# ru1ven/KeypointFusion

Hardware: AMD Instinct MI355X
Metric: RGB-D img/sec fwd (B=64, 256x256) (higher is better)
Workload: dtype f32; 1 GPU; KPFusion-convnext-tiny, depth+RGB UNet backbones forward, B=64/GPU 256x256 f32 (BASELINE configs[1]); batch_per_gpu=64, global_batch=64, input=256x256, parallelism=dp1 (batch shards, no collective)

## Files before the change

include/kpf.h:

```cpp
#ifndef KPF_H
#define KPF_H

#ifdef __cplusplus
extern "C" {
#endif

#define KPF_OK 0
#define KPF_EINVAL (-1)
#define KPF_ELAUNCH (-2)

#define KPF_DT_F32 0
#define KPF_DT_BF16 1
#define KPF_DT_F16 2
#define KPF_DT_F32_MMA_BF16 8
#define KPF_DT_F32_MMA_F16 9

#define KPF_ACT_RELU 1u
#define KPF_ACT_GELU 2u
#define KPF_RES_ADD 4u
#define KPF_RES_GAMMA 8u
#define KPF_RELU_AFTER_RES 16u
#define KPF_ACT_LEAKY 64u
#define KPF_IN_SPLIT 128u
#define KPF_W_SPLIT 512u
#define KPF_OUT_SPLIT 256u
#define KPF_OUT_NCHW 32u
#define KPF_ACT_GELU_SAVE 2048u
#define KPF_MMA_BF16 8192u
#define KPF_MMA_F16 16384u
#define KPF_PRO_LN 4096u
#define KPF_RES_GELU_GRAD 1024u

typedef struct kpf_conv_desc {
  int B, IH, IW, Cin;
  int in_ld, in_coff;
  int OH, OW, N;
  int KH, KW, sh, sw, ph, pw;
  int Kp;
  int out_ld, out_coff;
  int res_ld, res_coff;
  unsigned flags;
  float w_unscale;
  int tile_cfg;
  int groups;
  long w_gstride;
} kpf_conv_desc;

int kpf_conv2d_f32(const kpf_conv_desc* d, const float* in, const float* w, const float* bias,
                   const float* pro_scale, const float* pro_shift, const float* gamma, const float* res,
                   float* out, void* stream);

int kpf_dwconv7_ln_f32(const float* x, const float* w_dw, const float* b_dw, const float* ln_w, const float* ln_b,
                       float* y, int B, int H, int W, int C, float eps, void* stream);

int kpf_convnext_mlp_f32(const float* y, const float* x, const float* w1, const float* b1, const float* w2, const float* b2,
                         const float* gamma, float* out, long M, int C, void* stream);
int kpf_convnext_mlp_supported(int C);
int kpf_convnext_mlp_split_f32(const float* y_split, const float* x, const float* w1_split, const float* b1, float w1_unscale,
                               const float* w2_split_perm, const float* b2, float w2_unscale, const float* gamma, float* out, long M,
                               int C, void* stream);
int kpf_convnext_mlp_split_supported(int C);
int kpf_convnext_mlp_h16(const void* y, const void* x, const void* w1, const float* b1, const void* w2_chunks, const float* b2,
                         const float* gamma, void* out, long M, int C, int dtype, void* stream);
int kpf_convnext_mlp_h16_supported(int C);

int kpf_dwconv7_stats_h16(const void* x, const float* w_dw, const float* b_dw, void* y, float* stats, int B, int H, int W, int C, int dtype,
                          void* stream);
int kpf_dwconv7_stats_supported(int H, int W, int C);
long kpf_dwconv7_stats_floats(int B, int H, int W, int C);
int kpf_ln_apply_stats_h16(void* y, const float* stats, const float* ln_w, const float* ln_b, long rows, int C, float eps, int dtype, void* stream);
int kpf_ln_stats_merge(const float* stats, float* mean_rstd, long rows, int C, float eps, void* stream);

int kpf_layernorm_f32(const float* x, const float* w, const float* b, float* y, long rows, int C, float eps, void* stream);

int kpf_dwconv7_ln_split_f32(const float* x, const float* w_dw, const float* b_dw, const float* ln_w, const float* ln_b, float* y,
                             int B, int H, int W, int C, float eps, void* stream);
int kpf_layernorm_split_f32(const float* x, const float* w, const float* b, float* y, long rows, int C, float eps, void* stream);

int kpf_upsample2x_f32(const float* src, float* dst, int B, int H, int W, int C, int dst_ld, int dst_coff, void* stream);

int kpf_nchw_to_nhwc_f32(const float* src, float* dst, int B, int C, int H, int W, int Cpad, void* stream);

int kpf_nhwc_to_nchw_f32(const float* src, float* dst, int B, int C, int H, int W, int src_ld, int src_coff, void* stream);

int kpf_maxpool3x3s2_f32(const float* src, float* dst, int B, int H, int W, int C, void* stream);


int kpf_inv3x3_f32(const float* M, float* Minv, int B, int fused, void* stream);

int kpf_offset2joint_f32(const float* offset, const float* depth, const float* center, const float* Minv, const float* cube,
                         const float* cam, float* joint_uvd, float* joint_xyz, int B, int S, int F, float kernel,
                         int img_size, int flip, void* stream);

int kpf_img2pcl_top4_f32(const float* pcl, const float* depth, const float* center, const float* Minv, const float* cube,
                         const float* cam, float* closeness, int* index, float* img_xyz, int B, int N, int S, int F,
                         int img_size, int flip, void* stream);

int kpf_point_assemble_f32(const float* feat_d, const float* feat_rgb, const float* offset, const float* pcl,
                           const float* joint_xyz, const float* closeness, const int* index, float* A1, float* A2, int B,
                           int N, int P, float kernel, void* stream);

int kpf_softmax_pool_f32(const float* A1, const float* X, const float* joint_xyz, float* JA, int B, int N, void* stream);

// ... 368 lines not shown
                      int* bounds, double* M64, void* stream);

int kpf_prep_pcl_sample(const float* img, const float* center, const double* M64, const double* cube, const double* cam, const long long* seed, int B, int S,
                        int n, float* pcl, int* pcl_index, int* pcl_count, float* cand_pts, void* stream);

int kpf_prep_uncrop_f32(const float* joints, const float* center, const float* M, const float* cube, const float* cam, int B, int J, float* crop_px,
                        float* frame_px, void* stream);

int kpf_prep_set_stamps(void* stamps64 );

int kpf_eval_errors_f32(const float* const* stages, int S, const float* gt, const float* cube, const int* score_index, int B, int J, int Jsel, float* err,
                        void* stream);

int kpf_eval_accumulate(const float* err, const unsigned char* valid, const double* thresholds, int S, int B, int Jsel, int T, long long* n_samples,
                        long long* n_batches, double* sum_err, double* sum_pa, double* sum_batch_mean, double* sum_batch_pa_mean, long long* pck,
                        long long* pck_pa, void* stream);

int kpf_prep_crop_u16_indexed(const unsigned char* rgb, const unsigned short* depth, const int* frame_index, int F, const double* bbox, const double* cam,
                              const double* cube, int B, int Hs, int Ws, int x0, int y0, int H, int W, int S, float* img, float* img_rgb, float* center, float* M,
                              float* cube_out, float* cam_para, double* com, int* bounds, double* M64, void* stream);

int kpf_track_step_f32(const float* joints, const float* center, const float* M, const float* cube, const float* cam_para, const int* pcl_count, int B, int J,
                       int frame_w, int frame_h, float expansion, long long seed_stride, double* bbox, long long* seed, int* lost, float* crop_px,
                       float* frame_px, float* cam_mm, double* bbox_used, int* status, void* stream);

int kpf_prep_annot_u16(const unsigned char* rgb, const unsigned short* depth, const int* frame_index, int F, const float* joints_mm, const float* cam32,
                       const float* center_xyz, const unsigned char* mirror, const double* cube, int B, int J, int Hs, int Ws, int x0, int y0, int H, int W, int S,
                       float* img, float* img_rgb, float* center, float* M, float* cube_out, float* cam_para, double* com, int* bounds, double* M64, float* joint,
                       float* joint_img, double* cam64, void* stream);

int kpf_prep_uncrop_mirror_f32(const float* joints, const float* center, const float* M, const float* cube, const float* cam, const unsigned char* mirror,
                               int frame_w, int B, int J, float* crop_px, float* frame_px, void* stream);

int kpf_prep_augment_u16(const unsigned char* rgb, const unsigned short* depth, const int* frame_index, int F, const float* joints_mm, const float* cam32,
                         const float* center_xyz, const unsigned char* mirror, const double* cube, const int* mode, const double* off, const double* sc,
                         const double* rot, const double* rot_cs, const double* color, int B, int J, int Hs, int Ws, int x0, int y0, int H, int W, int S,
                         float* img, float* img_rgb, float* center, float* M, float* cube_out, float* cam_para, double* com, int* bounds, double* M64,
                         float* joint, float* joint_img, double* cam64, double* cube64, int* aug_status, void* stream);

int kpf_prep_aug_draw(long long* seed, int B, double sigma_com, double sigma_sc, double rot_range, double color_factor, long long seed_stride, int* mode,
                      double* off, double* sc, double* rot, double* rot_cs, double* color, void* stream);

int kpf_eval_mesh_f32(const float* pred, const float* gt, const float* pred_origin, const float* gt_origin, const double* thresholds, int T,
                      const double* f_thresholds, int Tf, int B, int V, float* err, float* nn, int* nn_idx, double* mean_err, int* pck_cnt, int* f_cnt,
                      void* stream);

int kpf_eval_mesh_accumulate(const float* err, const double* mean_err, const int* pck_cnt, const int* f_cnt, const unsigned char* valid, int B, int V, int T,
                             int Tf, long long* n_samples, long long* n_batches, double* sum_mean_err, double* sum_vert, long long* pck, double* sum_f,
                             void* stream);

int kpf_conv_num_tile_cfgs(void);

const char* kpf_last_error(void);
#define KPF_ABI_VERSION 32
int kpf_abi_version(void);

#ifdef __cplusplus
}
#endif
#endif
```

keypointfusion_amd/csrc/kpf_common.h:

```cpp
#pragma once
#include <hip/hip_runtime.h>
#include <stdarg.h>
#include <stdio.h>

#include "../../include/kpf.h"

typedef float f32x4 __attribute__((ext_vector_type(4)));
typedef _Float16 f16x4 __attribute__((ext_vector_type(4)));
typedef _Float16 f16x8 __attribute__((ext_vector_type(8)));

void kpf_set_error(const char* fmt, ...);

#define KPF_REQUIRE(cond, ...)    \
  do {                            \
    if (!(cond)) {                \
      kpf_set_error(__VA_ARGS__); \
      return KPF_EINVAL;          \
    }                             \
  } while (0)

static inline int kpf_check_launch(const char* what) {
  hipError_t e = hipGetLastError();
  if (e != hipSuccess) {
    kpf_set_error("%s: %s", what, hipGetErrorString(e));
    return KPF_ELAUNCH;
  }
  return KPF_OK;
}

#include <atomic>
constexpr int KPF_MAX_DEVICES = 64;
static inline bool kpf_raise_lds_limit(const void* kern, std::atomic<bool>* done) {
  int dev = 0;
  if (hipGetDevice(&dev) != hipSuccess || dev < 0 || dev >= KPF_MAX_DEVICES) return false;
  if (done[dev].load(std::memory_order_acquire)) return true;
  if (hipFuncSetAttribute(kern, hipFuncAttributeMaxDynamicSharedMemorySize, 160 * 1024) != hipSuccess) return false;
  done[dev].store(true, std::memory_order_release);
  return true;
}

void kpf_dw7_select_wgrad(int B, int H, int W, int C, bool raise_refused, kpf_dw7_plan* p, unsigned* grid_x);

static inline bool kpf_aligned16(const void* p) { return (reinterpret_cast<uintptr_t>(p) & 15u) == 0; }

__device__ __forceinline__ float wave_sum(float v) {
#pragma unroll
  for (int o = 32; o > 0; o >>= 1) v += __shfl_xor(v, o, 64);
  return v;
}
__device__ __forceinline__ float wave_max(float v) {
#pragma unroll
  for (int o = 32; o > 0; o >>= 1) v = fmaxf(v, __shfl_xor(v, o, 64));
  return v;
}

__host__ __device__ __forceinline__ unsigned hash32(unsigned x) {
  x ^= x >> 16;
  x *= 0x7feb352dU;
  x ^= x >> 15;
  x *= 0x846ca68bU;
  x ^= x >> 16;
  return x;
}

__device__ __forceinline__ void kpf_uncrop_joint(const float* __restrict__ j, const float* __restrict__ center, const float* __restrict__ M,
                                                 const float* __restrict__ cube, const float* __restrict__ cam, float* crop3, float* frame3,
                                                 double mirror_w = -1.0) {
#pragma clang fp contract(off)
  double m[9];
  for (int k = 0; k < 9; ++k) m[k] = (double)M[k];
  const double x = (double)j[0] * ((double)cube[0] / 2.0) + (double)center[0];
  const double y = (double)j[1] * ((double)cube[1] / 2.0) + (double)center[1];
  const double z = (double)j[2] * ((double)cube[2] / 2.0) + (double)center[2];
  const double u = x * (double)cam[0] / z + (double)cam[2], v = y * (double)cam[1] / z + (double)cam[3];
  const double cu = u * m[0] + v * m[1] + m[2], cv = u * m[3] + v * m[4] + m[5];
  crop3[0] = (float)cu;
  crop3[1] = (float)cv;
  crop3[2] = (float)z;
  const double c00 = m[4] * m[8] - m[5] * m[7], c01 = m[2] * m[7] - m[1] * m[8], c02 = m[1] * m[5] - m[2] * m[4];
  const double c10 = m[5] * m[6] - m[3] * m[8], c11 = m[0] * m[8] - m[2] * m[6], c12 = m[2] * m[3] - m[0] * m[5];
  const double c20 = m[3] * m[7] - m[4] * m[6], c21 = m[1] * m[6] - m[0] * m[7], c22 = m[0] * m[4] - m[1] * m[3];
  const double det = m[0] * c00 + m[1] * c10 + m[2] * c20;
  const double h0 = (cu * c00 + cv * c01 + c02) / det, h1 = (cu * c10 + cv * c11 + c12) / det, h2 = (cu * c20 + cv * c21 + c22) / det;
  const double fu = h0 / h2;
  frame3[0] = (float)(mirror_w >= 0.0 ? (mirror_w - 1.0) - fu : fu);
  frame3[1] = (float)(h1 / h2);
  frame3[2] = (float)z;
}

typedef __bf16 bf16_t;
typedef _Float16 f16_t;
typedef __bf16 bf16x4 __attribute__((ext_vector_type(4)));
typedef __bf16 bf16x8 __attribute__((ext_vector_type(8)));

// ... 39 lines not shown
```

keypointfusion_amd/csrc/kpf_conv.hip:

```cpp
#include "kpf_common.h"
#include <stdlib.h>
#include <type_traits>

namespace {

struct ConvArgs {
  const float* in;
  const float* w;
  const float* bias;
  const float* ps;
  const float* pt;
  const float* gamma;
  const float* res;
  float* out;
  int M, N, K, Kp;
  int IH, IW, Cin, in_ld, in_coff;
  int OH, OW, ohow, KH, KW, sh, sw, ph, pw;
  int out_ld, out_coff, res_ld, res_coff;
  const float* zero;
  float w_unscale;
  unsigned flags;
  int tilesN, nblk;
  int vec;
  int dbg;
// ... 1418 lines not shown
  KPF_REQUIRE(!(fl & KPF_RES_GELU_GRAD) || ((fl & KPF_RES_ADD) && !(fl & (KPF_RES_GAMMA | KPF_RELU_AFTER_RES | KPF_OUT_NCHW))), "kpf_conv2d_f32: RES_GELU_GRAD goes with RES_ADD alone");
  KPF_REQUIRE(!(fl & KPF_ACT_GELU_SAVE) || ((fl & KPF_ACT_GELU) && !(fl & (KPF_RES_ADD | KPF_OUT_NCHW)) && res && kpf_aligned16(res) && d->res_coff >= 0 && d->res_coff + d->N <= d->res_ld),
              "kpf_conv2d_f32: ACT_GELU_SAVE goes with ACT_GELU and a second output buffer in the res slot (res_ld / res_coff describe it)");
  KPF_REQUIRE((long)d->B * d->OH * d->OW < (1l << 31) && (long)d->B * d->IH * d->IW < (1l << 31), "kpf_conv2d_f32: too many pixels");

  ConvArgs a;
  a.in = in; a.w = w; a.bias = bias; a.ps = pro_scale; a.pt = pro_shift; a.gamma = gamma; a.res = res; a.out = out;
  a.M = d->B * d->OH * d->OW; a.N = d->N; a.K = d->KH * d->KW * d->Cin; a.Kp = d->Kp;
  a.IH = d->IH; a.IW = d->IW; a.Cin = d->Cin; a.in_ld = d->in_ld; a.in_coff = d->in_coff;
  a.OH = d->OH; a.OW = d->OW; a.ohow = d->OH * d->OW; a.KH = d->KH; a.KW = d->KW;
  a.sh = d->sh; a.sw = d->sw; a.ph = d->ph; a.pw = d->pw;
  a.out_ld = d->out_ld; a.out_coff = d->out_coff; a.res_ld = d->res_ld; a.res_coff = d->res_coff;
  {
    static const float* zero_of_dev[64] = {nullptr};
    int dev = 0;
    if (hipGetDevice(&dev) != hipSuccess || dev < 0 || dev >= 64) dev = 0;
    if (!zero_of_dev[dev]) {
      void* p = nullptr;
      if (hipGetSymbolAddress(&p, HIP_SYMBOL(kpf_zero16)) != hipSuccess || !p) {
        kpf_set_error("kpf_conv2d_f32: cannot resolve the zero page");
        return KPF_ELAUNCH;
      }
      zero_of_dev[dev] = static_cast<const float*>(p);
    }
    a.zero = zero_of_dev[dev];
  }
  a.flags = fl; a.tilesN = 0; a.nblk = 0; a.dbg = 0; a.skew = 0; a.st_policy = 0;
  {
    static const int st_mb = []() { const char* e = getenv("KPF_F32_ST_MB"); return e ? atoi(e) : 0; }();
    if (st_mb > 0 && (long)d->B * d->OH * d->OW * d->N * 4 >= (long)st_mb * 1000000) a.st_policy = 2;
  }
  a.w_unscale = (fl & (KPF_IN_SPLIT | KPF_W_SPLIT)) ? d->w_unscale : 1.0f;
  if (fl & (KPF_IN_SPLIT | KPF_W_SPLIT))
    KPF_REQUIRE(d->w_unscale > 0.f && d->Cin % 32 == 0 && d->in_coff % 4 == 0, "kpf_conv2d_f32: split operands need w_unscale > 0 and Cin %% 32 == 0 (Cin=%d)", d->Cin);
  if (fl & KPF_IN_SPLIT) KPF_REQUIRE(d->in_coff % 32 == 0 && d->in_ld % 32 == 0 && !pro_scale, "kpf_conv2d_f32: split activations need in_ld, in_coff multiples of 32 and no operand prologue");
  if (fl & KPF_OUT_SPLIT)
    KPF_REQUIRE(d->N % 32 == 0 && d->out_coff % 32 == 0 && d->out_ld % 32 == 0 && !(fl & KPF_OUT_NCHW),
                "kpf_conv2d_f32: split output needs N, out_ld, out_coff multiples of 32 (N=%d ld=%d coff=%d)", d->N, d->out_ld, d->out_coff);
  a.vec = (d->out_ld % 4 == 0 && d->out_coff % 4 == 0 && (!(fl & KPF_RES_ADD) || (d->res_ld % 4 == 0 && d->res_coff % 4 == 0))) ? 1 : 0;
  a.groups = d->groups > 1 ? d->groups : 1; a.g_in = a.g_out = 0; a.g_w = 0;
  if (a.groups > 1) {
    KPF_REQUIRE(!(fl & (KPF_RES_GAMMA | KPF_OUT_NCHW | KPF_IN_SPLIT | KPF_W_SPLIT | KPF_OUT_SPLIT)) && !pro_scale && d->w_gstride % 4 == 0,
                "kpf_conv2d_f32: a grouped launch takes no layer scale / prologue / NCHW output / split operands, and needs w_gstride %% 4 == 0");
    KPF_REQUIRE(d->in_coff + d->groups * d->Cin <= d->in_ld && d->out_coff + d->groups * d->N <= d->out_ld, "kpf_conv2d_f32: the groups' channel slices exceed the pixel stride");
    KPF_REQUIRE(!(fl & (KPF_RES_ADD | KPF_ACT_GELU_SAVE)) || d->res_coff + d->groups * d->N <= d->res_ld,
                "kpf_conv2d_f32: the groups' residual / saved pre-activation slices exceed the pixel stride");
    a.g_in = d->Cin; a.g_out = d->N; a.g_w = d->w_gstride;
    if ((d->out_coff + d->N) % 4 || ((fl & KPF_RES_ADD) && (d->res_coff + d->N) % 4)) a.vec = 0;
  }
  const bool is1x1 = d->KH == 1 && d->KW == 1 && d->sh == 1 && d->sw == 1 && d->ph == 0 && d->pw == 0 &&
                     d->IH == d->OH && d->IW == d->OW && d->Cin % 32 == 0 && d->Kp == d->Cin;
  hipStream_t st = reinterpret_cast<hipStream_t>(stream);

  int best = 0;
  double bc = 1e30;
  static const int forced = []() { const char* e = getenv("KPF_FORCE_CFG"); return e ? atoi(e) : -1; }();
  for (int i = 0; i < (int)(sizeof(kCfgs) / sizeof(kCfgs[0])); ++i) {
    const double c = cfg_cost(kCfgs[i], a.M, a.N, a.groups);
    if (c < bc) { bc = c; best = i; }
  }
  const bool f32_arith = !(fl & (KPF_IN_SPLIT | KPF_W_SPLIT));
  const bool gelu1x1 = f32_arith && is1x1 && (fl & KPF_ACT_GELU) && !(fl & KPF_ACT_GELU_SAVE) && !pro_scale && d->groups <= 1;
  if (gelu1x1 && a.M >= 1024 && a.N >= 512) {
    auto rounds_cost = [&](int bm, int bn, double pen) { return (double)((((long)(a.M + bm - 1) / bm) * ((a.N + bn - 1) / bn) + 255) / 256) * bm * bn * pen; };
    const double c0 = rounds_cost(128, 128, 1.00), c8 = rounds_cost(256, 128, 0.97);
    best = c0 <= c8 ? 0 : 8;
  }
  if (f32_arith && best < 9 && a.Kp >= 512) {
    const long bb = ((a.M + kCfgs[best].bm - 1) / kCfgs[best].bm) * ((a.N + kCfgs[best].bn - 1) / kCfgs[best].bn) * a.groups;
    if (bb < 256 && (long)((a.M + 31) / 32) * ((a.N + 63) / 64) * a.groups >= 512) best = 7;
  }
  if ((fl & (KPF_IN_SPLIT | KPF_W_SPLIT)) && !(fl & KPF_RES_ADD) && !pro_scale && (best == 0 || best == 8)) best = 13;
  if ((fl & (KPF_IN_SPLIT | KPF_W_SPLIT)) && !pro_scale && a.Kp >= 1024) {
    const long blocks = ((a.M + kCfgs[best < 9 ? best : 0].bm - 1) / kCfgs[best < 9 ? best : 0].bm) *
                        ((a.N + kCfgs[best < 9 ? best : 0].bn - 1) / kCfgs[best < 9 ? best : 0].bn);
    const long blocks64 = ((a.M + 63) / 64) * ((a.N + 63) / 64);
    if (best < 9 && blocks <= 512 && blocks64 >= 512) best = 16;
  }
  if (forced >= 0) best = forced;
  if (d->tile_cfg > 0) {
    KPF_REQUIRE(d->tile_cfg <= KPF_NUM_TILE_CFGS, "kpf_conv2d_f32: tile_cfg %d out of range", d->tile_cfg);
    best = d->tile_cfg - 1;
  }
#ifdef KPF_FAST_BUILD
  return launch_cfg<4, 4, 2, 2>(a, is1x1, st);
#else
  switch (best) {
    case 0: return launch_cfg<4, 4, 2, 2>(a, is1x1, st);
    case 1: return launch_cfg<4, 3, 2, 2>(a, is1x1, st);
    case 2: return launch_cfg<2, 4, 4, 1>(a, is1x1, st);
    case 3: return launch_cfg<4, 3, 4, 1>(a, is1x1, st);
    case 4: return launch_cfg<2, 7, 4, 1>(a, is1x1, st);
    case 5: return launch_cfg<2, 4, 2, 2>(a, is1x1, st);
    case 6: return launch_cfg<2, 2, 2, 2>(a, is1x1, st);
    case 8: return launch_cfg<4, 4, 4, 2>(a, is1x1, st);
    case 9: return launch_cfg<4, 4, 4, 2, 3>(a, is1x1, st);
    case 10: return launch_cfg<4, 4, 2, 2>(a, is1x1, st);
    case 11: return launch_cfg<4, 3, 2, 2>(a, is1x1, st);
    case 12: return launch_cfg<2, 4, 4, 1, 3>(a, is1x1, st);
    case 13: return launch_cfg<4, 4, 2, 2, 1>(a, is1x1, st);
    case 14: return launch_cfg<4, 3, 2, 2, 1>(a, is1x1, st);
    case 15: return launch_cfg<2, 4, 4, 1, 1>(a, is1x1, st);
    case 16: return launch_cfg<2, 2, 2, 2, 1>(a, is1x1, st);
    case 17: return launch_cfg<4, 6, 2, 2>(a, is1x1, st);
    default: return launch_cfg<2, 1, 1, 4>(a, is1x1, st);
  }
// ... 16 lines not shown
```

keypointfusion_amd/lib.py:

```python
import ctypes as C
import os

_HERE = os.path.dirname(os.path.abspath(__file__))
LIB_PATH = os.environ.get("KPF_LIB_PATH") or os.path.join(_HERE, "libkpf_hip.so")

KPF_ACT_RELU = 1
KPF_ACT_GELU = 2
KPF_RES_ADD = 4
KPF_RES_GAMMA = 8
KPF_RELU_AFTER_RES = 16
KPF_RES_GELU_GRAD = 1024
KPF_ACT_GELU_SAVE = 2048
KPF_PRO_LN = 4096
KPF_DT_F32_MMA_BF16, KPF_DT_F32_MMA_F16 = 8, 9
KPF_MMA_BF16, KPF_MMA_F16 = 8192, 16384
KPF_OUT_NCHW = 32
KPF_ACT_LEAKY = 64
KPF_IN_SPLIT = 128
KPF_OUT_SPLIT = 256
KPF_W_SPLIT = 512
KPF_DT_F32, KPF_DT_BF16, KPF_DT_F16 = 0, 1, 2
ABI_VERSION = 32


class ConvDesc(C.Structure):
    _fields_ = [(n, C.c_int) for n in (
        "B", "IH", "IW", "Cin", "in_ld", "in_coff", "OH", "OW", "N", "KH", "KW", "sh", "sw", "ph", "pw", "Kp",
        "out_ld", "out_coff", "res_ld", "res_coff")] + [("flags", C.c_uint), ("w_unscale", C.c_float), ("tile_cfg", C.c_int), ("groups", C.c_int), ("w_gstride", C.c_long)]


class PackDesc(C.Structure):
    _fields_ = [("src", C.c_void_p), ("dst", C.c_void_p)] + [(n, C.c_int) for n in (
        "N", "Cin", "KH", "KW", "mode", "n_pad", "Kp", "rows", "src_dtype", "dst_dtype", "first_block", "reserved")]


class AdamwDesc(C.Structure):
    _fields_ = [("p", C.c_void_p), ("g", C.c_void_p), ("m", C.c_void_p), ("v", C.c_void_p), ("n", C.c_long), ("first_block", C.c_int), ("reserved", C.c_int)]


class WgradGroupDesc(C.Structure):
    _fields_ = [("dy", C.c_void_p), ("x", C.c_void_p), ("dw", C.c_void_p), ("db", C.c_void_p), ("M", C.c_int), ("N", C.c_int), ("K", C.c_int), ("first_block", C.c_int), ("sps", C.c_int), ("ldy", C.c_int)]


class ColsumDesc(C.Structure):
    _fields_ = [("part", C.c_void_p), ("dw", C.c_void_p), ("db", C.c_void_p), ("nblk", C.c_int), ("C", C.c_int), ("first_block", C.c_int), ("reserved", C.c_int)]


class WgradReduceDesc(C.Structure):
    _fields_ = [("part", C.c_void_p), ("dbpart", C.c_void_p), ("dw", C.c_void_p), ("db", C.c_void_p), ("g_ws", C.c_long)] + [
        (n, C.c_int) for n in "S N K Cin KHW nkb ndb groups Cin_out N_out kind first_block".split()]


class ManoFitCfg(C.Structure):
    _fields_ = [("iters", C.c_int)] + [(n, C.c_float) for n in "lr_pose lr_shape lr_trans beta1 beta2 eps lambda_shape lambda_pose".split()] + [
        ("init_trans", C.c_int), ("joint_map", C.c_int * 21)]


class ManoFitMeshCfg(C.Structure):
    _fields_ = ManoFitCfg._fields_ + [("lambda_verts", C.c_float)]


class ManoFitGnCfg(C.Structure):
    _fields_ = [("iters", C.c_int)] + [(n, C.c_float) for n in "mu nu lambda_shape lambda_pose".split()] + [("init_trans", C.c_int), ("joint_map", C.c_int * 21)]


class ManoFitMeshGnCfg(C.Structure):
    _fields_ = ManoFitGnCfg._fields_ + [("lambda_verts", C.c_float)]


class WgradPlan(C.Structure):
    _fields_ = [(n, C.c_int) for n in "family vn vk tiles_n tiles_k S sps writes_dw".split()] + [("ws_floats", C.c_long)]


KPF_WGRAD_FAMILY = ("f32", "r16", "direct", "h16s", "h16")
KPF_WGRAD_FORM = {"f32_2x2": 1, "f32_2x4": 2, "f32_4x2": 3, "f32_4x4": 4, "h16s": 5, "h16": 6}


class Dw7Plan(C.Structure):
    _fields_ = [(n, C.c_int) for n in "family px rows taps_lds lg nt nchk cq S rows_per_chunk raise_lds reserved".split()] + [
        (n, C.c_long) for n in "blocks lds_bytes ws_floats".split()]


KPF_DW7_OP = {"ln": 0, "fwd": 1, "wgrad": 2}
KPF_DW7_FAMILY = ("tile", "wave", "wide", "two_launch", "tiny", "conv", "wgrad_lds", "wgrad_reg")

_P = C.c_void_p
_SIGS = {
    "kpf_conv2d_f32": [C.POINTER(ConvDesc), _P, _P, _P, _P, _P, _P, _P, _P, _P],
    "kpf_dwconv7_ln_f32": [_P, _P, _P, _P, _P, _P, C.c_int, C.c_int, C.c_int, C.c_int, C.c_float, _P],
    "kpf_layernorm_f32": [_P, _P, _P, _P, C.c_long, C.c_int, C.c_float, _P],
    "kpf_layernorm_split_f32": [_P, _P, _P, _P, C.c_long, C.c_int, C.c_float, _P],
    "kpf_dwconv7_ln_split_f32": [_P, _P, _P, _P, _P, _P, C.c_int, C.c_int, C.c_int, C.c_int, C.c_float, _P],
    "kpf_upsample2x_f32": [_P, _P, C.c_int, C.c_int, C.c_int, C.c_int, C.c_int, C.c_int, _P],
    "kpf_nchw_to_nhwc_f32": [_P, _P, C.c_int, C.c_int, C.c_int, C.c_int, C.c_int, _P],
    "kpf_nhwc_to_nchw_f32": [_P, _P, C.c_int, C.c_int, C.c_int, C.c_int, C.c_int, C.c_int, _P],
    "kpf_maxpool3x3s2_f32": [_P, _P, C.c_int, C.c_int, C.c_int, C.c_int, _P],
    "kpf_inv3x3_f32": [_P, _P, C.c_int, C.c_int, _P],
    "kpf_offset2joint_f32": [_P] * 8 + [C.c_int, C.c_int, C.c_int, C.c_float, C.c_int, C.c_int, _P],
    "kpf_img2pcl_top4_f32": [_P] * 9 + [C.c_int] * 6 + [_P],
    "kpf_point_assemble_f32": [_P] * 9 + [C.c_int, C.c_int, C.c_int, C.c_float, _P],
    "kpf_softmax_pool_f32": [_P, _P, _P, _P, C.c_int, C.c_int, _P],
    "kpf_ball_group_f32": [_P, _P, _P, _P, C.c_int, _P, _P, C.c_int, C.c_int, C.c_float, C.c_float, C.c_float, _P],
    "kpf_group_max_f32": [_P, _P, C.c_long, C.c_int, C.c_int, C.c_int, C.c_int, _P],
    "kpf_ball_group_stacked_f32": [_P, _P, _P, _P, C.c_int, _P, _P, _P, C.c_int, C.c_int, C.c_float, C.c_float, C.c_float, _P],
    "kpf_ball_group_bwd_f32": [_P, C.c_int, _P, _P, _P, _P, C.c_int, C.c_int, C.c_int, _P],
    "kpf_slices_sum_relu_forward": [_P, _P, C.c_long, C.c_int, C.c_int, C.c_int, _P],
    "kpf_slices_sum_relu_backward": [_P, _P, _P, _P, C.c_long, C.c_int, C.c_int, C.c_int, _P],
    "kpf_group_max_train_forward": [_P, _P, _P, C.c_long, C.c_int, C.c_int, _P],
    "kpf_group_max_train_backward": [_P, C.c_int, _P, _P, C.c_long, C.c_int, C.c_int, _P],
    "kpf_heat_gam_gate_f32": [_P, _P, _P, C.c_int] + [_P] * 10 + [C.c_int] * 4 + [_P],
    "kpf_gate_reduce_f32": [_P, _P, _P, _P, _P, C.c_int, C.c_int, _P],
    "kpf_tr_encoder_f32": [_P, C.c_int, C.c_int, _P, _P, _P, _P, C.c_int, C.c_int, _P],
    "kpf_xattn_layer_f32": [_P, _P, _P, _P, C.c_int, C.c_int, C.c_int, _P],
    "kpf_conv2d_h16": [C.POINTER(ConvDesc), _P, _P, _P, _P, _P, _P, _P, _P, C.c_int, _P],
    "kpf_conv2d_h16_uses_8ph": [C.POINTER(ConvDesc), C.c_int],
    "kpf_conv2d_h16_ln_fold_supported": [C.POINTER(ConvDesc)],
    "kpf_dwconv7_ln_h16": [_P, _P, _P, _P, _P, _P, C.c_int, C.c_int, C.c_int, C.c_int, C.c_float, C.c_int, _P],
    "kpf_layernorm_h16": [_P, C.c_int, _P, _P, _P, C.c_int, C.c_long, C.c_int, C.c_float, _P],
    "kpf_upsample2x_h16": [_P, _P, C.c_int, C.c_int, C.c_int, C.c_int, C.c_int, C.c_int, C.c_int, _P],
    "kpf_cast_h16_f32": [_P, C.c_int, _P, C.c_long, C.c_int, C.c_int, C.c_int, _P],
    "kpf_cast_f32_h16": [_P, _P, C.c_int, C.c_long, _P],
    "kpf_convnext_mlp_f32": [_P] * 8 + [C.c_long, C.c_int, _P],
    "kpf_convnext_mlp_supported": [C.c_int],
    "kpf_convnext_mlp_split_f32": [_P, _P, _P, _P, C.c_float, _P, _P, C.c_float, _P, _P, C.c_long, C.c_int, _P],
    "kpf_convnext_mlp_split_supported": [C.c_int],
    "kpf_convnext_mlp_h16": [_P] * 8 + [C.c_long, C.c_int, C.c_int, _P],
    "kpf_convnext_mlp_h16_supported": [C.c_int],
    "kpf_dwconv7_stats_h16": [_P, _P, _P, _P, _P, C.c_int, C.c_int, C.c_int, C.c_int, C.c_int, _P],
    "kpf_dwconv7_stats_supported": [C.c_int, C.c_int, C.c_int],
    "kpf_ln_apply_stats_h16": [_P, _P, _P, _P, C.c_long, C.c_int, C.c_float, C.c_int, _P],
    "kpf_ln_stats_merge": [_P, _P, C.c_long, C.c_int, C.c_float, _P],
    "kpf_cbam_channel_gate_f32": [_P] * 7 + [C.c_int] * 4 + [_P],
    "kpf_cbam_spatial_gate_f32": [_P, _P, _P, C.c_float, C.c_float, _P, _P, C.c_int, C.c_int, C.c_int, C.c_int, _P],
    "kpf_cbam_apply_f32": [_P] * 5 + [C.c_int] * 3 + [_P],
    "kpf_maxpool2x2_f32": [_P, _P, C.c_int, C.c_int, C.c_int, C.c_int, _P],
    "kpf_upnearest2x_add_f32": [_P, _P, _P, C.c_int, C.c_int, C.c_int, C.c_int, _P],
    "kpf_mano_forward_f32": [_P, C.c_int, _P, C.c_int] + [_P] * 10 + [C.c_int, _P],
    "kpf_mano_backward_f32": [_P, C.c_int, _P, C.c_int] + [_P] * 10 + [_P, C.c_int, _P, C.c_int, C.c_int, _P],
    "kpf_mano_fit_f32": [_P] * 8 + [C.POINTER(ManoFitCfg)] + [_P] * 8 + [C.c_int, _P],
    "kpf_mano_fit_mesh_f32": [_P] * 10 + [C.POINTER(ManoFitMeshCfg)] + [_P] * 8 + [C.c_int, _P],
    "kpf_mano_fit_gn_f32": [_P] * 8 + [C.POINTER(ManoFitGnCfg)] + [_P] * 10 + [C.c_int, _P],
    "kpf_mano_fit_mesh_gn_f32": [_P] * 10 + [C.POINTER(ManoFitMeshGnCfg)] + [_P] * 11 + [C.c_int, _P],
    "kpf_mano_assoc_f32": [_P, _P, _P, C.c_float, _P, _P, _P, _P, C.c_int, C.c_int, _P],
    "kpf_mano_normals_f32": [_P, _P, C.c_int, C.c_float, _P, C.c_int, _P],
    "kpf_mano_assoc_vis_f32": [_P, _P, _P, _P, C.c_float, C.c_float, _P, _P, _P, _P, _P, C.c_int, C.c_int, _P],
    "kpf_mano_assoc_vis_mask_f32": [_P, _P, _P, _P, _P, C.c_float, C.c_float, _P, _P, _P, _P, _P, C.c_int, C.c_int, _P],
    "kpf_mano_raster_f32": [_P, _P, C.c_int, _P, _P, C.c_int, C.c_int, C.c_float, _P, _P, _P, _P, _P, C.c_int, _P],
    "kpf_mano_fit_mesh_gn_plane_f32": [_P] * 11 + [C.POINTER(ManoFitMeshGnCfg)] + [_P] * 11 + [C.c_int, _P],
    "kpf_tr_encoder_weight_floats": [C.c_int],
    "kpf_conv_num_tile_cfgs": [],
    "kpf_xattn_weight_floats": [],
    "kpf_bn_train_forward": [_P, C.c_int, _P, _P, _P, C.c_int, _P, _P, _P, _P, C.c_float, C.c_float, C.c_int, _P, C.c_long, C.c_long, C.c_int, _P],
    "kpf_bn_train_backward": [_P, _P, _P, C.c_int, C.c_int, _P, _P, _P, _P, _P, _P, _P, C.c_int, _P, C.c_long, C.c_long, C.c_int, _P],
    "kpf_dwconv7_f32": [_P, _P, _P, _P, C.c_int, C.c_int, C.c_int, C.c_int, _P],
    "kpf_dwconv7_add_f32": [_P, _P, _P, _P, _P, C.c_int, C.c_int, C.c_int, C.c_int, _P],
    "kpf_conv2d_wgrad": [_P, _P, C.c_int] + [_P] * 3 + [C.c_long] + [C.c_int] * 18 + [C.POINTER(WgradReduceDesc), _P],
    "kpf_dwconv7_wgrad": [_P] * 5 + [C.c_long] + [C.c_int] * 4 + [C.POINTER(WgradReduceDesc), _P],
    "kpf_wgrad_reduce_multi": [C.POINTER(WgradReduceDesc), C.c_int, _P],
    "kpf_conv2d_wgrad_plan": [C.c_int, C.c_int, C.c_long, C.c_int, C.c_int, C.c_int, C.c_int, C.POINTER(WgradPlan)],
    "kpf_dwconv7_plan": [C.c_int] * 7 + [C.POINTER(Dw7Plan)],
    "kpf_conv2d_wgrad_force_form": [C.c_int],
    "kpf_row_gather_cols_f32": [_P, C.c_long, C.c_long, C.c_long, _P, _P, _P, C.c_int, C.c_int, C.c_int, C.c_int, C.c_int, _P],
    "kpf_bn_ssr_forward": [_P] * 7 + [C.c_float, C.c_float, _P, C.c_long, C.c_long, C.c_int, C.c_int, C.c_int, _P],
    "kpf_bn_ssr_backward": [_P] * 10 + [C.c_long, C.c_long, C.c_int, C.c_int, C.c_int, _P],
    "kpf_bn_relu_gmax_forward": [_P] * 8 + [C.c_float, C.c_float, _P, C.c_long, C.c_long, C.c_int, C.c_int, _P],
    "kpf_bn_relu_gmax_backward": [_P, C.c_int] + [_P] * 9 + [C.c_long, C.c_long, C.c_int, C.c_int, _P],
    "kpf_bn2_add_relu_forward": [_P] * 12 + [C.c_float, C.c_float, _P, C.c_long, C.c_long, C.c_int, _P],
    "kpf_bn2_add_relu_backward": [_P] * 14 + [C.c_long, C.c_long, C.c_int, _P],
# ... 131 lines not shown
```

Baseline: 3544 img/s.

## Add persistent streaming 1x1 conv kernel with LDS-resident weights for large-M f32

Adds a persistent f32 1x1-convolution kernel for large pixel counts (M >= 65536) with small channel counts (Kp <= 128, N <= 192). It keeps the whole weight matrix in LDS, or in registers when small enough, and streams input tiles through a three-slot LDS ring using async global-to-LDS loads. Blocks are capped at the CU count and interleaved across XCDs. The aim is to avoid reloading weights per tile and to overlap input fetches with MFMA work on these memory-bound layers. In exchange it adds many template instantiations and a separate epilogue path that must match the generic kernel's semantics.

```diff
diff --git a/include/kpf.h b/include/kpf.h
--- a/include/kpf.h
+++ b/include/kpf.h
@@ -49,6 +49,7 @@
 int kpf_conv2d_f32(const kpf_conv_desc* d, const float* in, const float* w, const float* bias,
                    const float* pro_scale, const float* pro_shift, const float* gamma, const float* res,
                    float* out, void* stream);
+int kpf_conv2d_f32_streams(const kpf_conv_desc* d, int has_prologue);
 
 int kpf_dwconv7_ln_f32(const float* x, const float* w_dw, const float* b_dw, const float* ln_w, const float* ln_b,
                        float* y, int B, int H, int W, int C, float eps, void* stream);
@@ -523,7 +524,7 @@
 int kpf_conv_num_tile_cfgs(void);
 
 const char* kpf_last_error(void);
-#define KPF_ABI_VERSION 32
+#define KPF_ABI_VERSION 33
 int kpf_abi_version(void);
 
 #ifdef __cplusplus
diff --git a/keypointfusion_amd/csrc/kpf_common.h b/keypointfusion_amd/csrc/kpf_common.h
--- a/keypointfusion_amd/csrc/kpf_common.h
+++ b/keypointfusion_amd/csrc/kpf_common.h
@@ -40,6 +40,21 @@
 }
 
 void kpf_dw7_select_wgrad(int B, int H, int W, int C, bool raise_refused, kpf_dw7_plan* p, unsigned* grid_x);
+
+struct kpf_stream1x1_args {
+  const float* in;
+  const float* w;
+  const float* bias;
+  const float* ps;
+  const float* pt;
+  const float* res;
+  float* out;
+  int M, N, Kp;
+  int in_ld, in_coff, out_ld, out_coff, res_ld, res_coff;
+  unsigned flags;
+};
+bool kpf_stream1x1_admits(const kpf_conv_desc* d, bool has_prologue);
+int kpf_stream1x1_launch(const kpf_stream1x1_args& a, hipStream_t st);
 
 static inline bool kpf_aligned16(const void* p) { return (reinterpret_cast<uintptr_t>(p) & 15u) == 0; }
 
diff --git a/keypointfusion_amd/csrc/kpf_conv.hip b/keypointfusion_amd/csrc/kpf_conv.hip
--- a/keypointfusion_amd/csrc/kpf_conv.hip
+++ b/keypointfusion_amd/csrc/kpf_conv.hip
@@ -1494,6 +1494,14 @@
                      d->IH == d->OH && d->IW == d->OW && d->Cin % 32 == 0 && d->Kp == d->Cin;
   hipStream_t st = reinterpret_cast<hipStream_t>(stream);
 
+  if (kpf_stream1x1_admits(d, pro_scale != nullptr)) {
+    kpf_stream1x1_args s;
+    s.in = in; s.w = w; s.bias = bias; s.ps = pro_scale; s.pt = pro_shift; s.res = res; s.out = out;
+    s.M = a.M; s.N = a.N; s.Kp = a.Kp; s.in_ld = a.in_ld; s.in_coff = a.in_coff;
+    s.out_ld = a.out_ld; s.out_coff = a.out_coff; s.res_ld = a.res_ld; s.res_coff = a.res_coff; s.flags = fl;
+    return kpf_stream1x1_launch(s, st);
+  }
+
   int best = 0;
   double bc = 1e30;
   static const int forced = []() { const char* e = getenv("KPF_FORCE_CFG"); return e ? atoi(e) : -1; }();
diff --git a/keypointfusion_amd/csrc/kpf_stream1x1.hip b/keypointfusion_amd/csrc/kpf_stream1x1.hip
--- /dev/null
+++ b/keypointfusion_amd/csrc/kpf_stream1x1.hip
@@ -0,0 +1,326 @@
+#include "kpf_common.h"
+#include <stdlib.h>
+
+namespace {
+
+typedef __attribute__((address_space(3))) void lds_void_t;
+typedef __attribute__((address_space(1))) void gbl_void_t;
+
+constexpr int BK = 32;
+constexpr int NW = 8;
+constexpr int NSLOT = 3;
+constexpr int LDS_MAX = 160 * 1024;
+enum { S_LIN = 0, S_RES = 1 };
+
+template <int CA>
+__device__ __forceinline__ void wait_tile() {
+  asm volatile("s_waitcnt vmcnt(%0) lgkmcnt(0)" ::"n"(CA) : "memory");
+}
+
+template <int WM, int WN, int TN, int NK, bool HAS_PRO, int EPI>
+__global__ __launch_bounds__(64 * NW) void stream1x1_f32_kernel(const kpf_stream1x1_args a) {
+  static_assert(WM * WN == NW, "eight waves");
+  constexpr int BM = 16 * WM, BN = 16 * TN * WN;
+  constexpr int GPK = BM / 8;
+  constexpr int WPK = NW / GPK;
+  static_assert(GPK * WPK == NW, "a pixel tile's row groups divide the waves");
+
+  extern __shared__ __attribute__((aligned(16))) float lds[];
+  constexpr int nk = NK;
+  constexpr int ca = (nk + WPK - 1) / WPK;
+  const int slot_f = nk * BM * BK;
+  float* const Wp = lds;
+  float* const ring = Wp + nk * BN * BK;
+  float* const pro_s = ring + NSLOT * slot_f;
+  float* const pro_t = pro_s + a.Kp;
+
+  const int tid = threadIdx.x;
+  const int lane = tid & 63;
+  const int wave = __builtin_amdgcn_readfirstlane(tid >> 6);
+  const int wm = wave % WM, wn = wave / WM;
+  const int fr = lane & 15, fg = lane >> 4, rsw = (fr >> 1) & 7;
+
+  const int G = gridDim.x;
+  int lw = blockIdx.x;
+  {
+    const int q = G >> 3, r = G & 7, x = lw & 7, i = lw >> 3;
+    lw = (x < r ? x * (q + 1) : r * (q + 1) + (x - r) * q) + i;
+  }
+  const int ntiles = (a.M + BM - 1) / BM;
+  if (lw >= ntiles) return;
+  const int nmy = (ntiles - lw + G - 1) / G;
+  const int last = lw + (nmy - 1) * G;
+
+  const int sg = wave % GPK, sk0 = wave / GPK;
+  const int srow = 8 * sg + (lane >> 3);
+  const int skc = ((lane & 7) ^ ((srow >> 1) & 7)) << 2;
+  auto stage = [&](int tile, int slot) {
+    const int m = tile * BM + srow;
+    const int mc = m < a.M ? m : a.M - 1;
+    const float* src = a.in + (long)mc * a.in_ld + a.in_coff + skc;
+    float* dst = ring + slot * slot_f + 8 * sg * BK;
+#pragma unroll
+    for (int i = 0; i < ca; ++i) {
+      int kt = sk0 + WPK * i;
+      kt = kt < nk ? kt : nk - 1;
+      __builtin_amdgcn_global_load_lds((gbl_void_t*)(src + kt * BK), (lds_void_t*)(dst + kt * BM * BK), 16, 0, 0);
+    }
+  };
+
+  for (int idx = wave; idx < (BN / 8) * nk; idx += NW) {
+    const int g = idx % (BN / 8), kt = idx / (BN / 8);
+    const int row = 8 * g + (lane >> 3);
+    const int nc = row < a.N ? row : a.N - 1;
+    const int kc = ((lane & 7) ^ ((row >> 1) & 7)) << 2;
+    __builtin_amdgcn_global_load_lds((gbl_void_t*)(a.w + (long)nc * a.Kp + kt * BK + kc), (lds_void_t*)(Wp + (kt * BN + 8 * g) * BK), 16, 0, 0);
+  }
+  stage(lw, 0);
+  stage(nmy > 1 ? lw + G : last, 1);
+  if (HAS_PRO) {
+    for (int i = tid; i < a.Kp; i += 64 * NW) {
+      pro_s[i] = a.ps[i];
+      pro_t[i] = a.pt[i];
+    }
+  }
+  const f32x4 zero4 = {0.f, 0.f, 0.f, 0.f};
+  f32x4 bv[TN];
+  bool nval[TN];
+#pragma unroll
+  for (int i = 0; i < TN; ++i) {
+    const int nb = (wn * TN + i) * 16;
+    nval[i] = nb < a.N;
+    bv[i] = zero4;
+    if (a.bias && nval[i]) {
+#pragma unroll
+      for (int e = 0; e < 4; ++e) bv[i][e] = a.bias[nb + fg * 4 + e];
+    }
+  }
+#pragma unroll
+  for (int i = 0; i < TN; ++i) asm volatile("" : "+v"(bv[i]));
+  asm volatile("s_waitcnt vmcnt(0) lgkmcnt(0)" ::: "memory");
+  __builtin_amdgcn_s_barrier();
+  __builtin_amdgcn_sched_barrier(0);
+
+  const unsigned fl = a.flags;
+  const int xoff = (wm * 16 + fr) * BK;
+  const int woff = (wn * TN * 16 + fr) * BK;
+
+  constexpr bool WREG = 8 * NK * TN <= 96;
+  f32x4 wr[WREG ? 2 * NK : 1][TN];
+  f32x4 spr[HAS_PRO ? 2 * NK : 1], tpr[HAS_PRO ? 2 * NK : 1];
+#pragma unroll
+  for (int q = 0; q < 2 * NK; ++q) {
+    const int sc = (((4 * (q & 1) + fg) ^ rsw) << 2);
+    if constexpr (WREG) {
+#pragma unroll
+      for (int i = 0; i < TN; ++i) wr[q][i] = *reinterpret_cast<const f32x4*>(Wp + woff + (q >> 1) * BN * BK + i * 16 * BK + sc);
+    }
+    if constexpr (HAS_PRO) {
+      spr[q] = *reinterpret_cast<const f32x4*>(pro_s + 16 * q + 4 * fg);
+      tpr[q] = *reinterpret_cast<const f32x4*>(pro_t + 16 * q + 4 * fg);
+    }
+  }
+
+  for (int j = 0; j < nmy; ++j) {
+    const int tile = lw + j * G;
+    const int slot = j % NSLOT;
+    const int m = tile * BM + wm * 16 + fr;
+    const bool mval = m < a.M;
+
+    f32x4 rv[EPI == S_RES ? TN : 1];
+    if constexpr (EPI == S_RES) {
+      const float* rrow = a.res + (long)(mval ? m : a.M - 1) * a.res_ld + a.res_coff + fg * 4;
+#pragma unroll
+      for (int i = 0; i < TN; ++i) rv[i] = *reinterpret_cast<const f32x4*>(rrow + (nval[i] ? (wn * TN + i) * 16 : 0));
+    }
+    stage(j + 2 < nmy ? tile + 2 * G : last, (j + 2) % NSLOT);
+    __builtin_amdgcn_sched_barrier(0);
+
+    f32x4 acc[TN];
+#pragma unroll
+    for (int i = 0; i < TN; ++i) acc[i] = zero4;
+    const float* xs = ring + slot * slot_f + xoff;
+    const float* ws = Wp + woff;
+    auto read_frags = [&](int q, f32x4& xf, f32x4(&wf)[TN]) {
+      const int sc = (((4 * (q & 1) + fg) ^ rsw) << 2);
+      xf = *reinterpret_cast<const f32x4*>(xs + (q >> 1) * BM * BK + sc);
+      if constexpr (!WREG) {
+#pragma unroll
+        for (int i = 0; i < TN; ++i) wf[i] = *reinterpret_cast<const f32x4*>(ws + (q >> 1) * BN * BK + i * 16 * BK + sc);
+      }
+    };
+    auto landed = [&](f32x4& xf, f32x4(&wf)[TN]) {
+      asm volatile("" : "+v"(xf));
+      if constexpr (!WREG) {
+#pragma unroll
+        for (int i = 0; i < TN; ++i) asm volatile("" : "+v"(wf[i]));
+      }
+    };
+    auto mma = [&](int q, f32x4 xf, const f32x4(&wf)[TN]) {
+      if constexpr (HAS_PRO) {
+#pragma unroll
+        for (int e = 0; e < 4; ++e) xf[e] = fmaxf(fmaf(xf[e], spr[q][e], tpr[q][e]), 0.f);
+      }
+#pragma unroll
+      for (int e = 0; e < 4; ++e)
+#pragma unroll
+        for (int i = 0; i < TN; ++i) acc[i] = __builtin_amdgcn_mfma_f32_16x16x4f32(WREG ? wr[WREG ? q : 0][i][e] : wf[i][e], xf[e], acc[i], 0, 0, 0);
+    };
+    f32x4 xa, xb, wa[TN], wb[TN];
+    read_frags(0, xa, wa);
+#pragma unroll
+    for (int kt = 0; kt < nk; ++kt) {
+      landed(xa, wa);
+      read_frags(2 * kt + 1, xb, wb);
+      __builtin_amdgcn_sched_barrier(0);
+      mma(2 * kt, xa, wa);
+      __builtin_amdgcn_sched_barrier(0);
+      landed(xb, wb);
+      if (kt + 1 < nk) read_frags(2 * kt + 2, xa, wa);
+      __builtin_amdgcn_sched_barrier(0);
+      mma(2 * kt + 1, xb, wb);
+      __builtin_amdgcn_sched_barrier(0);
+    }
+
+    __builtin_amdgcn_sched_barrier(0);
+    wait_tile<ca>();
+    __builtin_amdgcn_s_barrier();
+    __builtin_amdgcn_sched_barrier(0);
+
+    if constexpr (EPI == S_RES) {
+#pragma unroll
+      for (int i = 0; i < TN; ++i) asm volatile("" : "+v"(rv[i]));
+    }
+#pragma unroll
+    for (int i = 0; i < TN; ++i) {
+      f32x4 v = acc[i];
+      if constexpr (EPI == S_RES) {
+#pragma unroll
+        for (int e = 0; e < 4; ++e) {
+          float y = v[e] + bv[i][e];
+          y += rv[i][e];
+          if (fl & KPF_RELU_AFTER_RES) y = fmaxf(y, 0.f);
+          v[e] = y;
+        }
+      } else {
+#pragma unroll
+        for (int e = 0; e < 4; ++e) {
+          const float y = v[e] + bv[i][e];
+          v[e] = (fl & KPF_ACT_RELU) ? fmaxf(y, 0.f) : y;
+        }
+      }
+      if (nval[i] && mval) *reinterpret_cast<f32x4*>(a.out + (long)m * a.out_ld + a.out_coff + (wn * TN + i) * 16 + fg * 4) = v;
+    }
+  }
+  asm volatile("s_waitcnt vmcnt(0)" ::: "memory");
+}
+
+size_t lds_bytes(int bm, int bn, int Kp, bool pro) { return ((size_t)(bn + NSLOT * bm) * Kp + (pro ? 2 * Kp : 0)) * sizeof(float); }
+
+struct Geo {
+  int wm, tn;
+};
+Geo pick_geo(int N, int Kp, bool pro) {
+  static const int tn64[] = {2, 3, 4, 6}, tn32[] = {2, 3};
+  for (int tn : tn64)
+    if (32 * tn >= N) {
+      if (lds_bytes(64, 32 * tn, Kp, pro) <= (size_t)LDS_MAX) return {4, tn};
+      break;
+    }
+  for (int tn : tn32)
+    if (64 * tn >= N) {
+      if (lds_bytes(32, 64 * tn, Kp, pro) <= (size_t)LDS_MAX) return {2, tn};
+      break;
+    }
+  return {0, 0};
+}
+
+int env_int(const char* name, int dflt) {
+  const char* e = getenv(name);
+  return e && *e ? atoi(e) : dflt;
+}
+
+template <int WM, int WN, int TN, int NK, bool HAS_PRO, int EPI>
+int launch_one(const kpf_stream1x1_args& a, int grid, hipStream_t st) {
+  void (*kern)(const kpf_stream1x1_args) = stream1x1_f32_kernel<WM, WN, TN, NK, HAS_PRO, EPI>;
+  static std::atomic<bool> lds_opt_in[KPF_MAX_DEVICES];
+  if (!kpf_raise_lds_limit(reinterpret_cast<const void*>(kern), lds_opt_in)) {
+    kpf_set_error("kpf_conv2d_f32: cannot raise the dynamic LDS limit (streaming 1x1)");
+    return KPF_ELAUNCH;
+  }
+  const size_t lds = lds_bytes(16 * WM, 16 * TN * WN, a.Kp, HAS_PRO);
+  hipLaunchKernelGGL(kern, dim3(grid), dim3(64 * NW), lds, st, a);
+  return kpf_check_launch("kpf_conv2d_f32");
+}
+
+template <int WM, int WN, int TN, int NK>
+int launch_epi(const kpf_stream1x1_args& a, int grid, hipStream_t st) {
+  if (a.flags & KPF_RES_ADD) return launch_one<WM, WN, TN, NK, false, S_RES>(a, grid, st);
+  if (a.ps) return launch_one<WM, WN, TN, NK, true, S_LIN>(a, grid, st);
+  return launch_one<WM, WN, TN, NK, false, S_LIN>(a, grid, st);
+}
+
+template <int WM, int WN, int TN>
+int launch_nk(const kpf_stream1x1_args& a, int grid, hipStream_t st) {
+  switch (a.Kp / BK) {
+    case 1: return launch_epi<WM, WN, TN, 1>(a, grid, st);
+    case 2: return launch_epi<WM, WN, TN, 2>(a, grid, st);
+    case 3: return launch_epi<WM, WN, TN, 3>(a, grid, st);
+    default: return launch_epi<WM, WN, TN, 4>(a, grid, st);
+  }
+}
+
+}
+
+constexpr int KPF_STREAM1X1_MIN_M_DEFAULT = 65536;
+
+bool kpf_stream1x1_admits(const kpf_conv_desc* d, bool has_prologue) {
+  if (!d) return false;
+  if (env_int("KPF_STREAM1X1", 1) == 0) return false;
+  const unsigned fl = d->flags;
+  const bool is1x1 = d->KH == 1 && d->KW == 1 && d->sh == 1 && d->sw == 1 && d->ph == 0 && d->pw == 0 && d->IH == d->OH && d->IW == d->OW &&
+                     d->Cin > 0 && d->Cin % 32 == 0 && d->Kp == d->Cin;
+  if (!is1x1 || d->Kp > 128 || d->N <= 0 || d->N > 192 || d->N % 16) return false;
+  if (fl & (KPF_IN_SPLIT | KPF_W_SPLIT | KPF_OUT_SPLIT | KPF_MMA_BF16 | KPF_MMA_F16)) return false;
+  if (fl & (KPF_ACT_GELU | KPF_ACT_GELU_SAVE | KPF_RES_GELU_GRAD | KPF_ACT_LEAKY | KPF_RES_GAMMA | KPF_OUT_NCHW)) return false;
+  if (d->groups > 1 || d->tile_cfg != 0) return false;
+  if (has_prologue && (fl & KPF_RES_ADD)) return false;
+  const bool vec = d->out_ld % 4 == 0 && d->out_coff % 4 == 0 && (!(fl & KPF_RES_ADD) || (d->res_ld % 4 == 0 && d->res_coff % 4 == 0));
+  if (!vec) return false;
+  if (getenv("KPF_FORCE_CFG") || env_int("KPF_F32_ST_MB", 0) > 0) return false;
+  const long M = (long)d->B * d->OH * d->OW;
+  if (M < env_int("KPF_STREAM1X1_MIN_M", KPF_STREAM1X1_MIN_M_DEFAULT)) return false;
+  return pick_geo(d->N, d->Kp, has_prologue).wm != 0;
+}
+
+extern "C" int kpf_conv2d_f32_streams(const kpf_conv_desc* d, int has_prologue) { return kpf_stream1x1_admits(d, has_prologue != 0) ? 1 : 0; }
+
+int kpf_stream1x1_launch(const kpf_stream1x1_args& a, hipStream_t st) {
+  const Geo g = pick_geo(a.N, a.Kp, a.ps != nullptr);
+  if (!g.wm) {
+    kpf_set_error("kpf_conv2d_f32: no streaming geometry for N=%d Kp=%d", a.N, a.Kp);
+    return KPF_EINVAL;
+  }
+  static int cus_of_dev[KPF_MAX_DEVICES] = {0};
+  int dev = 0;
+  if (hipGetDevice(&dev) != hipSuccess || dev < 0 || dev >= KPF_MAX_DEVICES) dev = 0;
+  if (!cus_of_dev[dev]) {
+    int n = 0;
+    if (hipDeviceGetAttribute(&n, hipDeviceAttributeMultiprocessorCount, dev) != hipSuccess || n <= 0) n = 256;
+    cus_of_dev[dev] = n;
+  }
+  const int bm = 16 * g.wm;
+  const int tiles = (a.M + bm - 1) / bm;
+  int grid = tiles < cus_of_dev[dev] ? tiles : cus_of_dev[dev];
+  const int forced = env_int("KPF_STREAM1X1_GRID", 0);
+  if (forced > 0) grid = forced < cus_of_dev[dev] ? forced : cus_of_dev[dev];
+  if (g.wm == 4) {
+    switch (g.tn) {
+      case 2: return launch_nk<4, 2, 2>(a, grid, st);
+      case 3: return launch_nk<4, 2, 3>(a, grid, st);
+      case 4: return launch_nk<4, 2, 4>(a, grid, st);
+      default: return launch_nk<4, 2, 6>(a, grid, st);
+    }
+  }
+  return g.tn == 2 ? launch_nk<2, 4, 2>(a, grid, st) : launch_nk<2, 4, 3>(a, grid, st);
+}
diff --git a/keypointfusion_amd/lib.py b/keypointfusion_amd/lib.py
--- a/keypointfusion_amd/lib.py
+++ b/keypointfusion_amd/lib.py
@@ -20,7 +20,7 @@
 KPF_OUT_SPLIT = 256
 KPF_W_SPLIT = 512
 KPF_DT_F32, KPF_DT_BF16, KPF_DT_F16 = 0, 1, 2
-ABI_VERSION = 32
+ABI_VERSION = 33
 
 
 class ConvDesc(C.Structure):
@@ -114,6 +114,7 @@
     "kpf_xattn_layer_f32": [_P, _P, _P, _P, C.c_int, C.c_int, C.c_int, _P],
     "kpf_conv2d_h16": [C.POINTER(ConvDesc), _P, _P, _P, _P, _P, _P, _P, _P, C.c_int, _P],
     "kpf_conv2d_h16_uses_8ph": [C.POINTER(ConvDesc), C.c_int],
+    "kpf_conv2d_f32_streams": [C.POINTER(ConvDesc), C.c_int],
     "kpf_conv2d_h16_ln_fold_supported": [C.POINTER(ConvDesc)],
     "kpf_dwconv7_ln_h16": [_P, _P, _P, _P, _P, _P, C.c_int, C.c_int, C.c_int, C.c_int, C.c_float, C.c_int, _P],
     "kpf_layernorm_h16": [_P, C.c_int, _P, _P, _P, C.c_int, C.c_long, C.c_int, C.c_float, _P],
```

New measurement: 3567 img/s (median of 6 runs). No clear change (+0.6%).
